# TencentARC/HOSNeRF

Hardware: AMD Instinct MI355X
Metric: train rays/sec (stage3: forward + losses + backward + gradient all-reduce + Adam; LPIPS term OFF in this line -- stages.stage3_with_lpips carries it) (higher is better)
Workload: dtype f32 (fp16/bf16 hi-lo split MFMA x3, fp32 accumulate)

## Files before the change

hosnerf_amd/csrc/hos_chain.hip:

```cpp
#include "hos_common.h"
#include "hos_gemm_common.h"

namespace {

typedef _Float16 h8 __attribute__((ext_vector_type(8)));
typedef _Float16 h2 __attribute__((ext_vector_type(2)));

constexpr int CT = 256;
constexpr int CROWS = 128;
constexpr int NL = 6;
constexpr int CW = 128;
constexpr int KSMAX = 12;
constexpr int CBUF = KSMAX * 2 * 1024;
constexpr int SKIP_LAYER = 4;

__host__ __device__ constexpr int ks_of(int l, bool fold = false) { return l == SKIP_LAYER ? 12 : ((fold && l == 0) ? 4 : 8); }
__host__ __device__ constexpr int layer_off(int l, bool fold = false) {
    int o = 0;
    for (int i = 0; i < l; ++i) o += 4 * ks_of(i, fold) * 2048;
    return o;
}
constexpr int WC_BYTES = layer_off(NL);
constexpr int W0H_LD = 64;

struct ChainArgs {
    const float* E; int lde;
    const float* PE; int ldpe;
    const float* x;
    const uint16_t* Wc;
    const float* aux;
    float* acts[NL]; int ldact;
    float* xyz;
    long P; const int* p_dev;
    unsigned int* range_flag;
};
constexpr int AUX_FLOATS = NL * CW + 3 * CW + 4;
constexpr int AUX_BYTES = (AUX_FLOATS * 4 + 15) & ~15;
constexpr int SMEM_BYTES = 2 * CBUF + AUX_BYTES;

__device__ __forceinline__ void dma16(const void* gsrc, void* ldst) {
    __builtin_amdgcn_global_load_lds((const __attribute__((address_space(1))) void*)gsrc,
                                     (__attribute__((address_space(3))) void*)ldst, 16, 0, 0);
}

__device__ __forceinline__ f32x16 mfma3(const h8& ah, const h8& al, const h8& bh, const h8& bl, f32x16 acc) {
    acc = __builtin_amdgcn_mfma_f32_32x32x16_f16(al, bh, acc, 0, 0, 0);
    acc = __builtin_amdgcn_mfma_f32_32x32x16_f16(ah, bl, acc, 0, 0, 0);
    acc = __builtin_amdgcn_mfma_f32_32x32x16_f16(ah, bh, acc, 0, 0, 0);
    return acc;
}

__device__ __forceinline__ void split_to(float x, _Float16& hi, _Float16& lo) {
    hi = (_Float16)__builtin_amdgcn_fmed3f(x, -65504.f, 65504.f);
    lo = (_Float16)(x - (float)hi);
}

__device__ __forceinline__ void load_split8(const float* p, h8& hi, h8& lo) {
    const float4 a = *reinterpret_cast<const float4*>(p);
    const float4 b = *reinterpret_cast<const float4*>(p + 8);
    const float v[8] = {a.x, a.y, a.z, a.w, b.x, b.y, b.z, b.w};
#pragma unroll
    for (int c = 0; c < 8; ++c) { _Float16 h, l; split_to(v[c], h, l); hi[c] = h; lo[c] = l; }
}

#define CH_RD128(DST, ADDR, OFF) asm volatile("ds_read_b128 %0, %1 offset:%2" : "=v"(DST) : "v"(ADDR), "n"(OFF))

template <bool FOLD>
__global__ __launch_bounds__(CT, 2) void chain128_kernel(ChainArgs a) {
    extern __shared__ __attribute__((aligned(16))) char smem[];
    char* const wbuf = smem;
    float* const s_aux = reinterpret_cast<float*>(smem + 2 * CBUF);
    const int t = threadIdx.x, lane = t & 63, wave = t >> 6;
    const int r = lane & 31, hh = lane >> 5;
    long P = a.P;
    if (a.p_dev) P = min(P, (long)*a.p_dev);
    for (int i = t; i < AUX_FLOATS; i += CT) s_aux[i] = a.aux[i];
    const long ntiles = (P + CROWS - 1) / CROWS;
    if ((long)blockIdx.x >= ntiles) return;

    const unsigned voff = (unsigned)(wave * 1024 + lane * 16);
    auto issue_round = [&](int l, int ob, int parity, int q) {
        const int ks = ks_of(l, FOLD);
        const int lo = (l * 8 + (l > SKIP_LAYER ? 4 : 0) - ((FOLD && l > 0) ? 4 : 0)) * 4 * 2048;
        dma16(reinterpret_cast<const char*>(a.Wc) + lo + ob * ks * 2048 + voff + q * 4096, wbuf + parity * CBUF + wave * 1024 + q * 4096);
    };
    auto issue_chunk = [&](int l, int ob, int parity) {
        const int rounds = ks_of(l, FOLD) / 2;
        for (int q = 0; q < rounds; ++q) issue_round(l, ob, parity, q);
    };
    issue_chunk(0, 0, 0);
    const unsigned lds_base = (unsigned)(uintptr_t)(__attribute__((address_space(3))) char*)smem;

    bool big = false;
    for (long tile = blockIdx.x; tile < ntiles; tile += gridDim.x) {
        const long row = tile * CROWS + wave * 32 + r;
        const long lrow = row < P ? row : P - 1;
        const bool tile_full = (tile + 1) * CROWS <= P;
        h8 bh[KSMAX], bl[KSMAX];
        if constexpr (FOLD) {
            const float* pe = a.PE + (size_t)lrow * a.ldpe + 4 * hh;
#pragma unroll
            for (int s = 0; s < 4; ++s) load_split8(pe + 16 * s, bh[8 + s], bl[8 + s]);
#pragma unroll
            for (int s = 0; s < 8; ++s)
#pragma unroll
                for (int c = 0; c < 8; ++c) { bh[s][c] = (_Float16)0.f; bl[s][c] = (_Float16)0.f; }
        } else {
            const float* e = a.E + (size_t)lrow * a.lde + 4 * hh;
#pragma unroll
            for (int s = 0; s < 8; ++s) load_split8(e + 16 * s, bh[s], bl[s]);
#pragma unroll
            for (int s = 8; s < KSMAX; ++s)
#pragma unroll
                for (int c = 0; c < 8; ++c) { bh[s][c] = (_Float16)0.f; bl[s][c] = (_Float16)0.f; }
        }
        float part[3] = {0.f, 0.f, 0.f};
        int parity = 0;
#pragma unroll 1
// ... 264 lines not shown
```

hosnerf_amd/csrc/hos_gemm_common.h:

```cpp
#pragma once
#include "hos_common.h"

typedef float f32x16 __attribute__((ext_vector_type(16)));

enum Mode { MODE_FWD = 0, MODE_DGRAD = 1, MODE_WGRAD = 2 };

struct GemmArgs {
    const float* A0; int lda0; int kt0;
    const float* A1; int lda1;
    const float* B;  int ldb;
    float* C; int ldc;
    int M, N;
    int Mload, Nload;
    int red_limit;
    int nk;
    int kt_per_split;
    int tiles_m, tiles_n;
    const float* bias;
    const float* mask; int ldmask;
    float* aux; int aux_col; float p0, p1;
    float* db;
    int accumulate;
    int epi;
    const int* m_dev;
// ... 75 lines not shown
                v[0] += bias4.x; v[1] += bias4.y; v[2] += bias4.z; v[3] += bias4.w;
                const bool simple = (a.epi == HOS_EPI_NONE || a.epi == HOS_EPI_RELU);
                if (relu_bits != nullptr) {
                    uint32_t rb = *relu_bits;
#pragma unroll
                    for (int k = 0; k < 4; ++k) rb = __builtin_amdgcn_alignbit(rb, __float_as_uint(0.f - v[k]), 31);
                    *relu_bits = rb;
                }
                if (simple && full && c_vec) {
                    const float pre = (v[0] + v[1]) + (v[2] + v[3]);
                    if (a.epi == HOS_EPI_RELU) { v[0] = fmaxf(v[0], 0.f); v[1] = fmaxf(v[1], 0.f); v[2] = fmaxf(v[2], 0.f); v[3] = fmaxf(v[3], 0.f); }
                    big |= (fmaxf(fmaxf(fabsf(v[0]), fabsf(v[1])), fmaxf(fabsf(v[2]), fabsf(v[3]))) > HOS_RANGE_LIMIT) | (pre != pre);
                    *reinterpret_cast<float4*>(a.C + (size_t)row * a.ldc + colb) = make_float4(v[0], v[1], v[2], v[3]);
                } else {
#pragma unroll
                    for (int k = 0; k < 4; ++k) {
                        const int col = colb + k;
                        if (col >= a.N) break;
                        float x = v[k];
                        if (fwd_epilogue_value(a, x, row, col)) a.C[(size_t)row * a.ldc + col] = x;
                        if (simple) big |= !(fabsf(x) <= HOS_RANGE_LIMIT);
                    }
                }
            } else {
                if (a.mask != nullptr) {
                    if (full && m_vec) {
                        const float4 mk = *reinterpret_cast<const float4*>(a.mask + (size_t)row * a.ldmask + colb);
                        if (!(mk.x > 0.f)) v[0] = 0.f;
                        if (!(mk.y > 0.f)) v[1] = 0.f;
                        if (!(mk.z > 0.f)) v[2] = 0.f;
                        if (!(mk.w > 0.f)) v[3] = 0.f;
                    } else {
#pragma unroll
                        for (int k = 0; k < 4; ++k)
                            if (colb + k < a.N && !(a.mask[(size_t)row * a.ldmask + colb + k] > 0.f)) v[k] = 0.f;
                    }
                }
                float* dst = a.C + (size_t)row * a.ldc + colb;
                if (full && c_vec) {
                    float4 o = make_float4(v[0], v[1], v[2], v[3]);
                    if (a.accumulate) { const float4 p = *reinterpret_cast<const float4*>(dst); o.x += p.x; o.y += p.y; o.z += p.z; o.w += p.w; }
                    *reinterpret_cast<float4*>(dst) = o;
                } else {
#pragma unroll
                    for (int k = 0; k < 4; ++k)
                        if (colb + k < a.N) dst[k] = a.accumulate ? (dst[k] + v[k]) : v[k];
                }
            }
        }
        if (MODE == MODE_FWD && a.range_flag != nullptr && __builtin_amdgcn_ballot_w64(big) != 0 && lane == 0) atomicOr(a.range_flag, 1u);
    }
}

#define HOS_GEMM_FP32 0
#define HOS_GEMM_BF16X3 1
int hos_gemm3_launch(GemmArgs a, int mode, int splits, hipStream_t stream);
```

hosnerf_amd/human_nerf.py:

```python
from __future__ import annotations

import json
import math
import os
from types import SimpleNamespace
from typing import Dict, List, Optional

import numpy as np
import torch
import torch.nn as nn
import torch.nn.functional as F

from . import ops
from .flat import FlatModule, FlatStore, Region
from .mipnerf360 import select_state, _Lin

SMPL_PARENT = {1: 0, 2: 0, 3: 0, 4: 1, 5: 2, 6: 3, 7: 4, 8: 5, 9: 6, 10: 7, 11: 8, 12: 9, 13: 9, 14: 9, 15: 12,
               16: 13, 17: 14, 18: 16, 19: 17, 20: 18, 21: 19, 22: 20, 23: 21, 24: 23, 25: 22}


class Cfg(dict):

    def __getattr__(self, k):
        try:
# ... 423 lines not shown
        ops.embed_hannw(x, band_w, cond.reshape(-1), E, PE, rows_dev=rows_dev)
        if chain:
            key = id(specs)
            bufs = self._chain_bufs.get(key)
            if bufs is None or bufs[0].device != dev:
                bufs = self._chain_bufs[key] = ops.mlp_chain_buffers(dev)
            ws = [self._w(L) for L in specs]
            ops.mlp_chain_pack([w for w, _ in ws], [b_ for _, b_ in ws], bufs[0], bufs[1])
            acts = [torch.empty(Pn, 128, device=dev) for _ in range(6)]
            xyz = torch.empty(Pn, 3, device=dev)
            ops.mlp_chain128_fwd(E, PE, x, bufs[0], bufs[1], acts, xyz, rows_dev=rows_dev)
            return xyz, ((E, PE, acts, None) if save else None)
        acts = []
        h = E
        for i in range(6):
            L = specs[i]
            Wt, bt = self._w(L)
            out = torch.empty(Pn, 128, device=dev)
            if i == 4:
                ops.linear_fwd(h, 128, Wt, bt, 128, out, ops.EPI_RELU, A1=PE, K1=NR_LDPE, rows_dev=rows_dev)
            else:
                ops.linear_fwd(h, L.Kpad, Wt, bt, 128, out, ops.EPI_RELU, rows_dev=rows_dev)
            acts.append(out)
            h = out
        Wt, bt = self._w(specs[6])
        xyz = torch.empty(Pn, 3, device=dev)
        ops.linear_fwd(h, 128, Wt, bt, 3, xyz, ops.EPI_RESIDUAL, aux=x, rows_dev=rows_dev)
        return xyz, ((E, PE, acts, None) if save else None)

    def _canonical_fwd(self, cnl: torch.Tensor, state: int, save: bool, rows_dev=None):
        Pn = cnl.shape[0]
        dev = cnl.device
        embed = self._embeds.view(self.store.param)[state]
        fold = None
        if rows_dev is not None and not ops.thin_dgrad_rows(Pn):
            raise ValueError("_canonical_fwd(rows_dev=...): the row bound exists on the thin-kernel path only (ops.thin_dgrad_rows)")
        if ops.CNL_FOLD and ops.thin_dgrad_rows(Pn):
            fkey = ("cnl_fold",) + ops._stream_key(dev)
            fb = self._chain_bufs.get(fkey)
            if fb is None:
                fb = self._chain_bufs[fkey] = torch.empty(256 * (2 * CNL_NFP + 256 + 2), device=dev)
            fw = ops.cnl_fold_views(fb, 256, CNL_NFP, 256)
            (W0, b0), (W5, b5) = self._w(self._cnl[0]), self._w(self._cnl[5])
            ops.canonical_fold_pack(W0, b0, W5, b5, embed, 256, CNL_NF, 256, fw)
            E = torch.empty(Pn, CNL_NFP, device=dev)
            CAT = torch.empty(Pn, CNL_NFP + 256, device=dev)
            ops.embed_fourier(cnl, 10, ops.zero1(dev), E, CAT, rows_dev=rows_dev)
            fold = (fw, embed)
        else:
            E = torch.empty(Pn, CNL_LDE, device=dev)
            CAT = torch.empty(Pn, CNL_CAT, device=dev)
            CAT[:, CNL_CAT - 1].zero_()
            ops.embed_fourier(cnl, 10, embed, E, CAT, rows_dev=rows_dev)
        acts, bits = [], []
        h = E
        want_bits = save and ops.thin_dgrad_rows(Pn)
        for i in range(8):
            L = self._cnl[i]
            Wt, bt = self._w(L)
            K = L.Kpad
            if fold is not None and i in (0, 5):
                Wt, bt = (fold[0][0], fold[0][1]) if i == 0 else (fold[0][2], fold[0][3])
                K = Wt.shape[1]
            rb = ops.thin_relu_bits(Pn, dev) if (want_bits and K <= 320) else None
            if i == 4:
                ops.linear_fwd(h, K, Wt, bt, 256, CAT, ops.EPI_RELU, out_col0=CNL_NFP if fold is not None else 127, relu_bits=rb,
                               rows_dev=rows_dev)
                acts.append(CAT)
                h = CAT
            else:
                out = torch.empty(Pn, 256, device=dev)
                ops.linear_fwd(h, K, Wt, bt, 256, out, ops.EPI_RELU, relu_bits=rb, rows_dev=rows_dev)
                acts.append(out)
                h = out
            bits.append(rb)
        Wt, bt = self._w(self._cnl[8])
        raw = torch.empty(Pn, 4, device=dev)
        ops.linear_fwd(h, 256, Wt, bt, 4, raw, ops.EPI_SIGMOID_RELU4, rows_dev=rows_dev)
        return raw, ((E, acts, bits, fold) if save else None)

    def _nonrigid_bwd(self, specs: List[_LayerSpec], saved, x: torch.Tensor, band_w: torch.Tensor, g_xyz: torch.Tensor, rows_dev=None):
        E, PE, acts, fold = saved
        Pn, dev = x.shape[0], x.device

        def layer_bwd(dz, X, spec, N, K, out, relu_mask, w_col0=0, bias=True, override=None):
            if override is not None:
                Wt, gW, gb = override
            else:
                Wt, _ = self._w(spec)
                gW, gb = self._w(spec, grad=True)
            ops.linear_bwd_fused(dz, X, Wt, gW, gb if bias else None, N, K, out, relu_mask, w_col0=w_col0, rows_dev=rows_dev)
            return out

        dz6 = torch.empty(Pn, 32, device=dev)
        ops.slice_pad(g_xyz, 0, 3, dz6, rows_dev=rows_dev)
        if fold is not None:
            gfold = ops.zero_(ops.fold_grad_workspace(dev))
            gw0h, db0 = gfold[:128 * 64].view(128, 64), gfold[128 * 64:]
        if (fold is not None and ops.MLP_CHAIN_BWD and Pn >= ops.MLP_CHAIN_BWD_MIN_ROWS
                and ops.get_gemm_mode() != ops.GEMM_FP32):
            Wm = [self._w(L)[0] for L in specs]
            G = [self._w(L, grad=True) for L in specs]
            im = ops.mlp_chain_bwd_images(id(specs), (0, 1, 2), dev)
            ops.mlp_chain_bwd_pack([
                (0, 0, Wm[6], 0, 3, 128, im[0][0]), (0, 1, Wm[5], 0, 128, 128, im[0][1]),
                (1, 0, Wm[4], 128, 128, NR_LDPE, im[1][0]), (1, 1, Wm[4], 0, 128, 128, im[1][1]), (1, 2, Wm[3], 0, 128, 128, im[1][2]),
# ... 302 lines not shown
```

hosnerf_amd/ops.py:

```python
from __future__ import annotations

import os
import threading

import math
from typing import Optional, Tuple

import numpy as np
import torch

from . import _lib
from ._lib import call, ptr

EPS = 1.1920929e-07

EPI_NONE, EPI_RELU, EPI_DENSITY, EPI_RGB, EPI_NERF_HEAD, EPI_SIGMOID_RELU4, EPI_RESIDUAL = 0, 1, 2, 3, 4, 5, 6


def round_up(x: int, m: int) -> int:
    return (x + m - 1) // m * m


class KernelEvents:

# ... 334 lines not shown
    import ctypes
    for i in range(0, len(jobs), 8):
        js = jobs[i:i + 8]
        Wp = (ctypes.c_void_p * len(js))(*[ptr(j[2]) + 4 * j[3] for j in js])
        call("hos_mlp_chain_bwd_pack", len(js), _int_array([j[0] for j in js]), _int_array([j[1] for j in js]), Wp,
             _int_array([j[2].stride(0) for j in js]), _int_array([j[4] for j in js]), _int_array([j[5] for j in js]),
             (ctypes.c_void_p * len(js))(*[ptr(j[6], torch.int16) for j in js]))


def mlp_chain_bwd(cfg, dZ, X, images, dXout, dW, w_col0, db, N, K, rows_dev=None):
    import ctypes
    M = dZ.shape[0]
    S = len(X)
    need = int(_lib.load().hos_mlp_chain_bwd_ws_floats(cfg, M))
    ws = _bwd_workspace(dZ.device, need=need)
    flop = sum(4.0 * M * n * k for n, k in zip(N, K))
    _timed(f"mlp_chain_bwd{cfg}[M={M}]", flop, lambda: call(
        "hos_mlp_chain_bwd", cfg, ptr(dZ), dZ.stride(0), M, ptr(rows_dev, torch.int32), _ptr_array(list(X)), _int_array([x.stride(0) for x in X]),
        (ctypes.c_void_p * S)(*[ptr(im, torch.int16) for im in images]), _ptr_array(list(dXout)),
        _int_array([0 if o is None else o.stride(0) for o in dXout]),
        (ctypes.c_void_p * S)(*[ptr(g) + 4 * c for g, c in zip(dW, w_col0)]), _int_array([g.stride(0) for g in dW]),
        _ptr_array(list(db)), _int_array(N), _int_array(K), ptr(ws), ws.numel()))


def mlp_chain_buffers(device):
    lib = _lib.load()
    return (torch.empty(int(lib.hos_mlp_chain_weight_bytes()) // 2, dtype=torch.int16, device=device),
            torch.empty(int(lib.hos_mlp_chain_aux_floats()), device=device))


def mlp_chain_pack(weights, biases, planes, aux):
    import ctypes
    ldw = (ctypes.c_int * 7)(*[int(w.stride(0)) for w in weights])
    call("hos_mlp_chain_pack", _ptr_array(list(weights)), ldw, _ptr_array(list(biases)), ptr(planes, torch.int16), ptr(aux))


def mlp_chain_pack_fold(weights, biases, cond, nfeat, planes, aux, w0h):
    import ctypes
    ldw = (ctypes.c_int * 7)(*[int(w.stride(0)) for w in weights])
    call("hos_mlp_chain_pack_fold", _ptr_array(list(weights)), ldw, _ptr_array(list(biases)), ptr(cond), cond.numel(), nfeat,
         ptr(planes, torch.int16), ptr(aux), ptr(w0h))


def mlp_chain_unfold_grad(gw0h, db, cond, nfeat, gW0, gb0):
    call("hos_mlp_chain_unfold_grad", ptr(gw0h), ptr(db), ptr(cond), cond.numel(), nfeat, ptr(gW0), gW0.stride(0), ptr(gb0))


def mlp_chain128_fwd(E, PE, x, planes, aux, acts, xyz, rows_dev=None):
    P = x.shape[0]
    flop = 101120 if E is not None else 101120 - 128 * 64
    _timed(f"mlp_chain128{'' if E is not None else 'f'}[M={P}]", 2.0 * P * flop, lambda: call(
        "hos_mlp_chain128_fwd", ptr(E), 0 if E is None else E.stride(0), ptr(PE), PE.stride(0), ptr(x), ptr(planes, torch.int16), ptr(aux),
        _ptr_array(list(acts)), acts[0].stride(0), ptr(xyz), P, ptr(rows_dev, torch.int32)))


_RANGE_FLAG = {}
RANGE_GUARD = os.environ.get("HOS_RANGE_GUARD", "1") != "0"


def arm_range_flag(device) -> torch.Tensor:
    key = str(device)
    if key not in _RANGE_FLAG:
        _RANGE_FLAG[key] = torch.zeros(1, dtype=torch.int32, device=device)
    _lib.check(_lib.load().hos_set_range_flag(ptr(_RANGE_FLAG[key], torch.int32)), "hos_set_range_flag")
    return _RANGE_FLAG[key]


def range_events(device, reset: bool = True) -> int:
    flag = _RANGE_FLAG.get(str(device))
    if flag is None:
        return 0
    v = int(flag.item())
    if v and reset:
        flag.zero_()
    return v


_RANGE_SKIPS = {}
_RANGE_SKIPS_SEEN = {}


def range_guard_words(device):
    if not RANGE_GUARD:
        return None, None
    key = str(device)
    if key not in _RANGE_FLAG or key not in _RANGE_SKIPS:
        if torch.cuda.is_current_stream_capturing():
            return None, None
        arm_range_flag(device)
        _RANGE_SKIPS[key] = torch.zeros(2, dtype=torch.int32, device=device)
    return _RANGE_FLAG[key], _RANGE_SKIPS[key]


def range_skips(device, since_last_poll: bool = False) -> int:
    key = str(device)
    t = _RANGE_SKIPS.get(key)
    if t is None:
        return 0
    n = int(t[0].item())
    if since_last_poll:
        n, _RANGE_SKIPS_SEEN[key] = n - _RANGE_SKIPS_SEEN.get(key, 0), n
    return n


def guarded_forward(module, device, run):
    mode = getattr(module, "gemm_mode", None)
# ... 1279 lines not shown
```

include/hosrender.h:

```cpp
#ifndef HOSRENDER_H
#define HOSRENDER_H

#include <stdint.h>

#ifdef __cplusplus
extern "C" {
#endif

#define HOS_OK 0
#define HOS_E_ARG (-1)
#define HOS_E_ALIGN (-2)
#define HOS_E_SHAPE (-3)
#define HOS_E_NODEVICE (-4)

typedef void* hos_stream_t;

#define HOS_ABI_VERSION 101

int hos_version(void);
int hos_device_count(void);
const char* hos_error_string(int code);


#define HOS_GEMM_MODE_FP32 0
// ... 213 lines not shown
int hos_raw2outputs_bwd(const float* g_rgb, const float* g_weights, const float* rgbs, int rgb_ld,
                        const float* sigma, int sigma_ld, const float* z_vals, const float* rays_d,
                        const float* mask, const float* bgcolor, float last_dist, int B, int S,
                        float* g_rgbs, int g_rgb_ld, float* g_sigma, int g_sigma_ld, float* g_mask,
                        hos_stream_t stream);

int hos_merge_composite_fwd(const float* bkg_tdist, const float* bkg_rgb, const float* bkg_density,
                            const float* human_rgbsigma, const float* newsmpl_pts, const float* pts_mask,
                            const float* rays_o_bkg, const float* rays_d_bkg, const float* smpl_to_world,
                            const int32_t* tiny_d_flag, int B, int Sb, int Sh, float thre_fg,
                            float* rgb, int32_t* idx_fg, int32_t* total_order, float* human_weights_sorted,
                            float* z_human, hos_stream_t stream);
int hos_merge_composite_maps_fwd(const float* bkg_tdist, const float* bkg_rgb, const float* bkg_density,
                                 const float* human_rgbsigma, const float* newsmpl_pts, const float* pts_mask,
                                 const float* rays_o_bkg, const float* rays_d_bkg, const float* smpl_to_world,
                                 const int32_t* tiny_d_flag, int B, int Sb, int Sh, float thre_fg,
                                 float* rgb, int32_t* idx_fg, int32_t* total_order,
                                 float* acc, float* depth, float* rgb_human, float* acc_human,
                                 float* rgb_bkg, float* acc_bkg, hos_stream_t stream);
int hos_merge_composite_bwd(const float* g_rgb, const float* g_human_weights_sorted,
                            const float* bkg_tdist, const float* bkg_rgb, const float* bkg_density,
                            const float* human_rgbsigma, const float* newsmpl_pts, const float* pts_mask,
                            const float* rays_o_bkg, const float* rays_d_bkg, const float* smpl_to_world,
                            const int32_t* tiny_d_flag, int B, int Sb, int Sh, float thre_fg,
                            float* g_bkg_rgb, float* g_bkg_density, float* g_human_rgbsigma, float* g_pts_mask,
                            hos_stream_t stream);

long long hos_pose_refine_saved_floats(void);
long long hos_pose_refine_workspace_floats(void);
int hos_pose_refine_fwd(const float* posevec, const float* Rs, const float* Ts, const float* const* weights14,
                        int F, int K, int width, float* Rs_out, float* Ts_out, float* saved, hos_stream_t stream);
int hos_pose_refine_bwd(const float* g_Rs_out, const float* g_Ts_out, const float* posevec, const float* Rs,
                        const float* saved, const float* const* weights14, float* const* grads14, int F, int K, int width,
                        float* workspace, hos_stream_t stream);

int hos_motion_basis_fwd(const float* dst_Rs, const float* dst_Ts, const float* cnl_gtfms, int F, int K,
                         float* R_bwd, float* T_bwd, float* R_fwd, float* T_fwd, hos_stream_t stream);
int hos_motion_basis_bwd(const float* g_R_bwd, const float* g_T_bwd, const float* g_R_fwd, const float* g_T_fwd,
                         const float* dst_Rs, const float* dst_Ts, const float* cnl_gtfms, int F, int K,
                         float* g_dst_Rs, float* g_dst_Ts, hos_stream_t stream);

long long hos_mlp_chain_weight_bytes(void);
long long hos_mlp_chain_aux_floats(void);
int hos_mlp_chain_pack(const float* const* weights7, const int* ldw7, const float* const* biases7, void* chain_planes,
                       float* aux, hos_stream_t stream);
int hos_mlp_chain_pack_fold(const float* const* weights7, const int* ldw7, const float* const* biases7, const float* cond,
                            int ncond, int nfeat, void* chain_planes, float* aux, float* w0h, hos_stream_t stream);
int hos_mlp_chain_unfold_grad(const float* gw0h, const float* db, const float* cond, int ncond, int nfeat,
                              float* gW0, int ldw, float* gb0, hos_stream_t stream);
int hos_mlp_chain128_fwd(const float* E, int lde, const float* PE, int ldpe, const float* x, const void* chain_planes,
                         const float* aux, float* const* acts6, int ldact, float* xyz, int64_t P,
                         const int32_t* rows_dev, hos_stream_t stream);

int hos_mlp_chain_bwd_steps(int cfg);
long long hos_mlp_chain_bwd_image_bytes(int cfg, int step);
long long hos_mlp_chain_bwd_ws_floats(int cfg, int M);
int hos_mlp_chain_bwd_pack(int n, const int* cfg, const int* step, const float* const* W, const int* ldw, const int* N, const int* K,
                           void* const* image, hos_stream_t stream);
int hos_mlp_chain_bwd(int cfg, const float* dZ, int lddz, int M, const int32_t* rows_dev, const float* const* X, const int* ldx,
                      const void* const* images, float* const* dXout, const int* lddx, float* const* dW, const int* lddw,
                      float* const* db, const int* N, const int* K, float* ws, int64_t ws_floats, hos_stream_t stream);

long long hos_compact_workspace_ints(void);
int hos_compact_rows(const float* mask, float thr, const float* src_a, const float* src_b, int64_t P, int32_t* count,
                     int32_t* sel, float* out_a, float* out_b, int32_t* workspace, hos_stream_t stream);
int hos_scatter_rows(const float* src, const int32_t* sel, const int32_t* count, int64_t P, float* dst, hos_stream_t stream);

int hos_select_live_rays(const float* mask, float thr, int B, int S, int32_t* ray_ids, int32_t* flag, int32_t* rows_live,
                         hos_stream_t stream);
int hos_gather_rays(const float* src, const int32_t* ray_ids, const int32_t* rows_live, int B, int S, int C, float* dst,
                    hos_stream_t stream);
int hos_scatter_rays(const float* src, const int32_t* ray_ids, const int32_t* flag, const int32_t* rows_live, int B, int S,
                     int C, float* dst, hos_stream_t stream);

long long hos_train_losses_workspace_floats(void);
int hos_train_losses_fwd(const float* rgb, const float* target, long long n_rays, float mse_const, float mse_count,
                         const float* pts_prev, const float* weights, const float* ray_grid, const int32_t* fg,
                         const float* cam_prev, const float* intrinsics_prev, int S,
                         const float* observe, const float* deform, long long n_cyc, const int32_t* n_cyc_dev,
                         float w_mse, float w_flow, float w_cycle, float* workspace, float* out8,
                         hos_stream_t stream);
int hos_train_losses_bwd(const float* g_total, const float* out8, const float* rgb, const float* target, long long n_rays,
                         float mse_count, const float* pts_prev, const float* weights, const float* ray_grid,
                         const int32_t* fg, const float* cam_prev, const float* intrinsics_prev, int S,
                         const float* observe, const float* deform, long long n_cyc, const int32_t* n_cyc_dev,
                         float w_mse, float w_flow, float w_cycle,
                         float* g_rgb, float* g_pts_prev, float* g_weights, float* g_deform, hos_stream_t stream);

int hos_sumsq(const float* g, int64_t n, float* sumsq, hos_stream_t stream);
int hos_adam_step(float* p, const float* g, float* m, float* v, int64_t n, float lr, float beta1,
                  float beta2, float eps, int step, float grad_scale, const float* sumsq,
                  float max_norm, hos_stream_t stream);

int hos_adam_step_dyn(float* p, const float* g, float* m, float* v, int64_t n, const float* hyper,
                      float beta1, float beta2, float eps, float grad_scale, const float* sumsq,
                      float max_norm, hos_stream_t stream);

int hos_rowdot_lrelu_fwd(const float* x, const float* W, int ldw, const float* b, int N, int K, float slope, float* y,
                         hos_stream_t stream);
int hos_rowdot_lrelu_bwd(const float* g, const float* y, const float* x, const float* W, int ldw, int N, int K, float slope,
                         float* gW, int ldgw, float* gb, float* gx, hos_stream_t stream);
int hos_volume_softmax_fwd(const float* z, const float* prior, int C, long long V3, float* vol, hos_stream_t stream);
int hos_volume_softmax_bwd(const float* g_vol, const float* vol, int C, long long V3, float* gz, hos_stream_t stream);
int hos_volume_channel_last(const float* vol, int Kb, long long V3, float* vol_cl, hos_stream_t stream);
int hos_volume_pair_bwd(const float* g_vol, const float* g_cl, int C, int Kb, long long V3, float* g, hos_stream_t stream);
int hos_copy_or_zero_n(int n, float* const* dst, const float* const* src, const long long* count, hos_stream_t stream);
// ... 47 lines not shown
```

Measured before the change: 143,300.

## Fuse the 8-layer canonical MLP into one persistent chain256 kernel

Adds a persistent HIP kernel that runs the full 256-wide, 8-layer canonical NeRF MLP, including the skip layer and the 4-output head, inside one launch. Activations stay in registers as fp16 hi/lo splits, and weight tiles are double-buffered into LDS with global_load_lds DMA. When saving for backward it writes activations and packed ReLU sign bits. This replaces a sequence of per-layer GEMM launches and their activation round-trips through global memory. The cost is a large single-occupancy kernel (launch_bounds 1, big LDS footprint) and a weight repack on every forward call.

```diff
diff --git a/hosnerf_amd/csrc/hos_chain.hip b/hosnerf_amd/csrc/hos_chain.hip
--- a/hosnerf_amd/csrc/hos_chain.hip
+++ b/hosnerf_amd/csrc/hos_chain.hip
@@ -3,8 +3,7 @@
 
 namespace {
 
-typedef _Float16 h8 __attribute__((ext_vector_type(8)));
-typedef _Float16 h2 __attribute__((ext_vector_type(2)));
+using namespace hos_chainp;
 
 constexpr int CT = 256;
 constexpr int CROWS = 128;
@@ -37,33 +36,6 @@
 constexpr int AUX_FLOATS = NL * CW + 3 * CW + 4;
 constexpr int AUX_BYTES = (AUX_FLOATS * 4 + 15) & ~15;
 constexpr int SMEM_BYTES = 2 * CBUF + AUX_BYTES;
-
-__device__ __forceinline__ void dma16(const void* gsrc, void* ldst) {
-    __builtin_amdgcn_global_load_lds((const __attribute__((address_space(1))) void*)gsrc,
-                                     (__attribute__((address_space(3))) void*)ldst, 16, 0, 0);
-}
-
-__device__ __forceinline__ f32x16 mfma3(const h8& ah, const h8& al, const h8& bh, const h8& bl, f32x16 acc) {
-    acc = __builtin_amdgcn_mfma_f32_32x32x16_f16(al, bh, acc, 0, 0, 0);
-    acc = __builtin_amdgcn_mfma_f32_32x32x16_f16(ah, bl, acc, 0, 0, 0);
-    acc = __builtin_amdgcn_mfma_f32_32x32x16_f16(ah, bh, acc, 0, 0, 0);
-    return acc;
-}
-
-__device__ __forceinline__ void split_to(float x, _Float16& hi, _Float16& lo) {
-    hi = (_Float16)__builtin_amdgcn_fmed3f(x, -65504.f, 65504.f);
-    lo = (_Float16)(x - (float)hi);
-}
-
-__device__ __forceinline__ void load_split8(const float* p, h8& hi, h8& lo) {
-    const float4 a = *reinterpret_cast<const float4*>(p);
-    const float4 b = *reinterpret_cast<const float4*>(p + 8);
-    const float v[8] = {a.x, a.y, a.z, a.w, b.x, b.y, b.z, b.w};
-#pragma unroll
-    for (int c = 0; c < 8; ++c) { _Float16 h, l; split_to(v[c], h, l); hi[c] = h; lo[c] = l; }
-}
-
-#define CH_RD128(DST, ADDR, OFF) asm volatile("ds_read_b128 %0, %1 offset:%2" : "=v"(DST) : "v"(ADDR), "n"(OFF))
 
 template <bool FOLD>
 __global__ __launch_bounds__(CT, 2) void chain128_kernel(ChainArgs a) {
diff --git a/hosnerf_amd/csrc/hos_chain256.hip b/hosnerf_amd/csrc/hos_chain256.hip
--- /dev/null
+++ b/hosnerf_amd/csrc/hos_chain256.hip
@@ -0,0 +1,307 @@
+#include "hos_common.h"
+#include "hos_gemm_common.h"
+
+namespace {
+
+using namespace hos_chainp;
+
+typedef float f32x4 __attribute__((ext_vector_type(4)));
+typedef unsigned u32x4 __attribute__((ext_vector_type(4)));
+
+constexpr int CT = 256;
+constexpr int CROWS = 128;
+constexpr int NL = 8;
+constexpr int CW = 256;
+constexpr int NOB = CW / 32;
+constexpr int KSE = 4;
+constexpr int KSH = CW / 16;
+constexpr int KSMAX = KSH + KSE;
+constexpr int CBUF = KSMAX * 2048;
+constexpr int SKIP_LAYER = 5;
+constexpr int NOUT = 4;
+
+__host__ __device__ constexpr int ks_of(int l) { return l == 0 ? KSE : (l == SKIP_LAYER ? KSMAX : KSH); }
+__host__ __device__ constexpr int ks_before(int l) { return l == 0 ? 0 : KSE + KSH * (l - 1) + (l > SKIP_LAYER ? KSE : 0); }
+constexpr int WC_BYTES = NOB * ks_before(NL) * 2048;
+constexpr int AUX_FLOATS = NL * CW + NOUT * CW + NOUT;
+constexpr int AUX_BYTES = (AUX_FLOATS * 4 + 15) & ~15;
+constexpr int BITS_BYTES = 4 * 1024;
+constexpr int SMEM_BYTES = 2 * CBUF + AUX_BYTES + BITS_BYTES;
+
+struct Chain256Args {
+    const float* E; int lde;
+    const uint16_t* Wc;
+    const float* aux;
+    float* acts[NL]; int ldact[NL];
+    uint16_t* bits[NL];
+    float* raw;
+    long P; const int* p_dev;
+    unsigned int* range_flag;
+};
+
+template <int NS, int CS0, int SLOT0, bool EPI, typename F, typename G, typename H>
+__device__ __forceinline__ void run_steps(f32x16& acc, const h8 (&bh)[KSMAX], const h8 (&bl)[KSMAX], unsigned la, F&& issue, H&& pre, G&& epi) {
+    h8 fh[2], fl[2];
+    f32x4 bq = {0.f, 0.f, 0.f, 0.f};
+    CH_RD128(fh[0], la, (2 * CS0) * 1024);
+    CH_RD128(fl[0], la, (2 * CS0 + 1) * 1024);
+#pragma unroll
+    for (int s = 0; s < NS; ++s) {
+        if (EPI && s >= NS - 4) pre(s - (NS - 4), bq);
+        if (s < NS - 1) {
+            CH_RD128(fh[(s + 1) & 1], la, (2 * (CS0 + s) + 2) * 1024);
+            CH_RD128(fl[(s + 1) & 1], la, (2 * (CS0 + s) + 3) * 1024);
+            asm volatile("s_waitcnt lgkmcnt(2)" : "+v"(fh[s & 1]), "+v"(fl[s & 1]), "+v"(bq));
+        } else {
+            asm volatile("s_waitcnt lgkmcnt(0)" : "+v"(fh[0]), "+v"(fl[0]), "+v"(fh[1]), "+v"(fl[1]), "+v"(bq));
+        }
+        acc = mfma3(fh[s & 1], fl[s & 1], bh[SLOT0 + s], bl[SLOT0 + s], acc);
+        issue(CS0 + s);
+        if (EPI && s >= NS - 4) epi(s - (NS - 4), bq);
+    }
+}
+
+template <bool SAVE>
+__global__ __launch_bounds__(CT, 1) void chain256_kernel(Chain256Args a) {
+    extern __shared__ __attribute__((aligned(16))) char smem[];
+    char* const wbuf = smem;
+    float* const s_aux = reinterpret_cast<float*>(smem + 2 * CBUF);
+    const int t = threadIdx.x, lane = t & 63, wave = __builtin_amdgcn_readfirstlane(t >> 6);
+    const int r = lane & 31, hh = lane >> 5;
+    long P = a.P;
+    if (a.p_dev) P = min(P, (long)*a.p_dev);
+    for (int i = t; i < AUX_FLOATS; i += CT) s_aux[i] = a.aux[i];
+    const long ntiles = (P + CROWS - 1) / CROWS;
+    if ((long)blockIdx.x >= ntiles) return;
+
+    const unsigned voff = (unsigned)(wave * 1024 + lane * 16);
+    auto issue_round = [&](int l, int ob, int parity, int q) {
+        const unsigned off = (unsigned)((NOB * ks_before(l) + ob * ks_of(l)) * 2048 + q * 4096) + voff;
+        dma16(reinterpret_cast<const char*>(a.Wc) + off, wbuf + parity * CBUF + wave * 1024 + q * 4096);
+    };
+    for (int q = 0; q < KSE / 2; ++q) issue_round(0, 0, 0, q);
+    const unsigned lds_base = (unsigned)(uintptr_t)(__attribute__((address_space(3))) char*)smem;
+
+    const int thin_l0 = 32 * ((r >> 2) & 1) + (r & 3) + 4 * hh;
+    const int bits_shift = 12 - 4 * (r >> 3) + 16 * (r & 1);
+    const unsigned bits_la = lds_base + (unsigned)(2 * CBUF + AUX_BYTES + wave * 1024 + (thin_l0 >> 1) * 4);
+    const unsigned stage_la = lds_base + (unsigned)(2 * CBUF + AUX_BYTES + wave * 1024 + lane * 16);
+
+    float v_max = 0.f, pre_sum = 0.f;
+    for (long tile = blockIdx.x; tile < ntiles; tile += gridDim.x) {
+        const long row0 = tile * CROWS + wave * 32;
+        const long row = row0 + r;
+        const long lrow = row < P ? row : P - 1;
+        const bool wave_live = row0 < P;
+        h8 bh[KSMAX], bl[KSMAX];
+        {
+            const float* e = a.E + (size_t)lrow * a.lde + 4 * hh;
+#pragma unroll
+            for (int s = 0; s < KSE; ++s) load_split8(e + 16 * s, bh[KSH + s], bl[KSH + s]);
+#pragma unroll
+            for (int s = 0; s < KSH; ++s)
+#pragma unroll
+                for (int c = 0; c < 8; ++c) { bh[s][c] = (_Float16)0.f; bl[s][c] = (_Float16)0.f; }
+        }
+        float part[NOUT] = {0.f, 0.f, 0.f, 0.f};
+        int parity = 0;
+#pragma unroll 1
+        for (int l = 0; l < NL; ++l) {
+            const int ks = ks_of(l);
+            const unsigned bias_la = lds_base + (unsigned)(2 * CBUF + (l * CW + 4 * hh) * 4);
+            float* out = SAVE ? a.acts[l] + (size_t)lrow * a.ldact[l] + 4 * hh : nullptr;
+            if (SAVE) { const u32x4 z = {0u, 0u, 0u, 0u}; asm volatile("ds_write_b128 %0, %1" :: "v"(stage_la), "v"(z) : "memory"); }
+            f32x16 acc[NOB];
+            auto epi_bias = [&](int ob, int q, f32x4& b4) {
+                asm volatile("ds_read_b128 %0, %1" : "=v"(b4) : "v"(bias_la + (unsigned)((32 * ob + 8 * q) * 4)));
+            };
+            auto epi_bias_now = [&](int ob, int q, f32x4& b4) {
+                asm volatile("ds_read_b128 %0, %1\n\ts_waitcnt lgkmcnt(0)" : "=v"(b4) : "v"(bias_la + (unsigned)((32 * ob + 8 * q) * 4)));
+            };
+            auto epi_quad = [&](f32x16& A, int ob, int q, const f32x4& b4) {
+                const int n0 = 32 * ob + 8 * q;
+                const float p0 = A[4 * q + 0] + b4[0], p1 = A[4 * q + 1] + b4[1], p2 = A[4 * q + 2] + b4[2], p3 = A[4 * q + 3] + b4[3];
+                pre_sum += (p0 + p1) + (p2 + p3);
+                const float v0 = fmaxf(p0, 0.f), v1 = fmaxf(p1, 0.f), v2 = fmaxf(p2, 0.f), v3 = fmaxf(p3, 0.f);
+                A[4 * q + 0] = v0; A[4 * q + 1] = v1; A[4 * q + 2] = v2; A[4 * q + 3] = v3;
+                v_max = fmaxf(fmaxf(v_max, fmaxf(v0, v1)), fmaxf(v2, v3));
+                if (SAVE) {
+                    uint32_t nib = 0;
+                    nib = __builtin_amdgcn_alignbit(nib, __float_as_uint(0.f - p0), 31);
+                    nib = __builtin_amdgcn_alignbit(nib, __float_as_uint(0.f - p1), 31);
+                    nib = __builtin_amdgcn_alignbit(nib, __float_as_uint(0.f - p2), 31);
+                    nib = __builtin_amdgcn_alignbit(nib, __float_as_uint(0.f - p3), 31);
+                    asm volatile("ds_or_b32 %0, %1" :: "v"(bits_la + (unsigned)(ob * 128 + q * 16)), "v"(row < P ? nib << bits_shift : 0u) : "memory");
+                    if (row < P) *reinterpret_cast<float4*>(out + n0) = make_float4(v0, v1, v2, v3);
+                }
+            };
+#pragma unroll
+            for (int ob = 0; ob < NOB; ++ob) {
+#pragma unroll
+                for (int i = 0; i < 16; ++i) acc[ob][i] = 0.f;
+                if (SAVE && wave_live && ob >= 2) asm volatile("s_waitcnt vmcnt(4)" ::: "memory");
+                else if (SAVE && wave_live && ob == 0 && l > 0) asm volatile("s_waitcnt vmcnt(8)" ::: "memory");
+                else asm volatile("s_waitcnt vmcnt(0)" ::: "memory");
+                asm volatile("s_waitcnt lgkmcnt(0)\n\ts_barrier" ::: "memory");
+                int nl = l, nob = ob + 1;
+                if (nob == NOB) { nob = 0; nl = l + 1 == NL ? 0 : l + 1; }
+                const int nrounds = ks_of(nl) / 2;
+                const int npar = parity ^ 1;
+                const unsigned la = lds_base + (unsigned)(parity * CBUF + lane * 16);
+                parity ^= 1;
+                auto issue = [&](int q) { if (q < nrounds) issue_round(nl, nob, npar, q); };
+                auto pre = [&](int q, f32x4& b4) { if (ob > 0) epi_bias(ob - 1, q, b4); };
+                auto epi = [&](int q, const f32x4& b4) {
+                    if (q == 0) asm volatile("" ::: "memory");
+                    if (ob > 0) epi_quad(acc[ob > 0 ? ob - 1 : 0], ob - 1, q, b4);
+                };
+                auto none = [](int) {};
+                auto none2 = [](int, f32x4&) {};
+                if (l == 0) {
+                    run_steps<KSE, 0, KSH, false>(acc[ob], bh, bl, la, issue, none2, none2);
+                    for (int q = KSE; q < nrounds; ++q) issue_round(nl, nob, npar, q);
+                    asm volatile("" ::: "memory");
+                    if (ob > 0) {
+#pragma unroll
+                        for (int q = 0; q < 4; ++q) { f32x4 b4; epi_bias_now(ob - 1, q, b4); epi_quad(acc[ob - 1], ob - 1, q, b4); }
+                    }
+                } else {
+                    run_steps<KSH, 0, 0, true>(acc[ob], bh, bl, la, issue, pre, epi);
+                    if (ks == KSMAX) run_steps<KSE, KSH, KSH, false>(acc[ob], bh, bl, la, none, none2, none2);
+                }
+            }
+            asm volatile("" ::: "memory");
+#pragma unroll
+            for (int q = 0; q < 4; ++q) { f32x4 b4; epi_bias_now(NOB - 1, q, b4); epi_quad(acc[NOB - 1], NOB - 1, q, b4); }
+            const bool last = l == NL - 1;
+#pragma unroll
+            for (int ob = 0; ob < NOB; ++ob) {
+#pragma unroll
+                for (int tq = 0; tq < 2; ++tq) {
+                    h8 hi, lo;
+#pragma unroll
+                    for (int c = 0; c < 8; ++c) { _Float16 h_, l_; split_to(acc[ob][8 * tq + c], h_, l_); hi[c] = h_; lo[c] = l_; }
+                    bh[2 * ob + tq] = hi;
+                    bl[2 * ob + tq] = lo;
+                }
+            }
+            if (last) {
+                const float* w8 = s_aux + NL * CW + 4 * hh;
+#pragma unroll
+                for (int ob = 0; ob < NOB; ++ob)
+#pragma unroll
+                    for (int q = 0; q < 4; ++q)
+#pragma unroll
+                        for (int m = 0; m < NOUT; ++m) {
+                            const float4 w4 = *reinterpret_cast<const float4*>(w8 + m * CW + 32 * ob + 8 * q);
+                            part[m] += acc[ob][4 * q] * w4.x + acc[ob][4 * q + 1] * w4.y + acc[ob][4 * q + 2] * w4.z + acc[ob][4 * q + 3] * w4.w;
+                        }
+            }
+            if (SAVE) {
+                u32x4 w;
+                asm volatile("ds_read_b128 %0, %1\n\ts_waitcnt lgkmcnt(0)" : "=v"(w) : "v"(stage_la) : "memory");
+                if (wave_live) *reinterpret_cast<u32x4*>(reinterpret_cast<char*>(a.bits[l]) + (size_t)(row0 / 32) * 1024 + lane * 16) = w;
+            }
+        }
+#pragma unroll
+        for (int m = 0; m < NOUT; ++m) part[m] += __shfl_xor(part[m], 32, 64);
+        if (hh == 0 && row < P) {
+            const float* b8 = s_aux + NL * CW + NOUT * CW;
+            *reinterpret_cast<float4*>(a.raw + row * 4) = make_float4(sigmoid_f(part[0] + b8[0]), sigmoid_f(part[1] + b8[1]),
+                                                                      sigmoid_f(part[2] + b8[2]), fmaxf(part[3] + b8[3], 0.f));
+        }
+    }
+    asm volatile("s_waitcnt vmcnt(0)" ::: "memory");
+    if (a.range_flag != nullptr && __builtin_amdgcn_ballot_w64((v_max > HOS_RANGE_LIMIT) | (pre_sum != pre_sum)) != 0 && lane == 0) atomicOr(a.range_flag, 1u);
+}
+
+struct Pack256Args {
+    const float* W[NL + 1]; int ldw[NL + 1];
+    const float* b[NL + 1];
+    uint16_t* Wc; float* aux;
+};
+
+__global__ __launch_bounds__(256) void chain256_pack_kernel(Pack256Args p) {
+    const int l = blockIdx.y;
+    if (l == NL) {
+        for (int i = blockIdx.x * 256 + threadIdx.x; i < AUX_FLOATS; i += gridDim.x * 256) {
+            float v;
+            if (i < NL * CW) v = p.b[i / CW][i % CW];
+            else if (i < NL * CW + NOUT * CW) { const int j = i - NL * CW; v = p.W[NL][(size_t)(j / CW) * p.ldw[NL] + j % CW]; }
+            else v = p.b[NL][i - NL * CW - NOUT * CW];
+            p.aux[i] = v;
+        }
+        return;
+    }
+    const int ks = ks_of(l);
+    const int total = NOB * ks * 64 * 8;
+    uint16_t* dst = p.Wc + (size_t)NOB * ks_before(l) * 1024;
+    for (int e = blockIdx.x * 256 + threadIdx.x; e < total; e += gridDim.x * 256) {
+        const int c = e & 7, lane = (e >> 3) & 63, s = (e >> 9) % ks, ob = (e >> 9) / ks;
+        const int n = 32 * ob + (lane & 31);
+        int k = 16 * s + 8 * (c >> 2) + 4 * (lane >> 5) + (c & 3);
+        if (l == SKIP_LAYER) k = k < CW ? k + 16 * KSE : k - CW;
+        _Float16 hi, lo;
+        split_to(p.W[l][(size_t)n * p.ldw[l] + k], hi, lo);
+        const size_t o = (((size_t)(ob * ks + s) * 2) * 64 + lane) * 8 + c;
+        dst[o] = __builtin_bit_cast(uint16_t, hi);
+        dst[o + 64 * 8] = __builtin_bit_cast(uint16_t, lo);
+    }
+}
+
+template <bool SAVE>
+int chain256_launch(const Chain256Args& a, hipStream_t stream) {
+    static bool attr_set = false;
+    if (!attr_set) {
+        hipError_t e = hipFuncSetAttribute(reinterpret_cast<const void*>(&chain256_kernel<SAVE>), hipFuncAttributeMaxDynamicSharedMemorySize, SMEM_BYTES);
+        if (e != hipSuccess) return (int)e;
+        attr_set = true;
+    }
+    const long ntiles = (a.P + CROWS - 1) / CROWS;
+    constexpr int max_grid = 256;
+    const int grid = (int)(ntiles < max_grid ? ntiles : max_grid);
+    hipLaunchKernelGGL(chain256_kernel<SAVE>, dim3(grid), dim3(CT), SMEM_BYTES, stream, a);
+    return hos_launch_status();
+}
+
+}
+
+extern "C" long long hos_mlp_chain256_weight_bytes(void) { return WC_BYTES; }
+extern "C" long long hos_mlp_chain256_aux_floats(void) { return AUX_FLOATS; }
+
+extern "C" int hos_mlp_chain256_pack(const float* const* weights9, const int* ldw9, const float* const* biases9, void* chain_planes,
+                                     float* aux, hos_stream_t stream) {
+    if (!weights9 || !ldw9 || !biases9 || !chain_planes || !aux) return HOS_E_ARG;
+    Pack256Args p{};
+    for (int l = 0; l <= NL; ++l) {
+        if (!weights9[l] || !biases9[l]) return HOS_E_ARG;
+        if (ldw9[l] < (l == NL ? CW : 16 * ks_of(l))) return HOS_E_SHAPE;
+        p.W[l] = weights9[l]; p.ldw[l] = ldw9[l]; p.b[l] = biases9[l];
+    }
+    p.Wc = static_cast<uint16_t*>(chain_planes); p.aux = aux;
+    hipLaunchKernelGGL(chain256_pack_kernel, dim3(48, NL + 1), dim3(256), 0, static_cast<hipStream_t>(stream), p);
+    return hos_launch_status();
+}
+
+extern "C" int hos_mlp_chain256_canonical_fwd(const float* E, int lde, const void* chain_planes, const float* aux,
+                                              float* const* acts8, const int* ldact8, void* const* relu_bits8, float* raw,
+                                              int64_t P, const int32_t* rows_dev, hos_stream_t stream) {
+    if (!E || !chain_planes || !aux || !raw || P <= 0) return HOS_E_ARG;
+    if (lde < 16 * KSE || P > (int64_t)1 << 22) return HOS_E_SHAPE;
+    if ((lde & 3) || (((uintptr_t)E | (uintptr_t)chain_planes | (uintptr_t)raw) & 15u)) return HOS_E_ALIGN;
+    Chain256Args a{};
+    a.E = E; a.lde = lde; a.Wc = static_cast<const uint16_t*>(chain_planes); a.aux = aux; a.raw = raw;
+    a.P = P; a.p_dev = rows_dev; a.range_flag = hos_range_flag_ptr();
+    const bool save = acts8 != nullptr;
+    if (save) {
+        if (!ldact8 || !relu_bits8) return HOS_E_ARG;
+        for (int l = 0; l < NL; ++l) {
+            if (!acts8[l] || !relu_bits8[l]) return HOS_E_ARG;
+            if (ldact8[l] < CW) return HOS_E_SHAPE;
+            if ((ldact8[l] & 3) || (((uintptr_t)acts8[l] | (uintptr_t)relu_bits8[l]) & 15u)) return HOS_E_ALIGN;
+            a.acts[l] = acts8[l]; a.ldact[l] = ldact8[l]; a.bits[l] = static_cast<uint16_t*>(relu_bits8[l]);
+        }
+    }
+    hipStream_t s = static_cast<hipStream_t>(stream);
+    return save ? chain256_launch<true>(a, s) : chain256_launch<false>(a, s);
+}
diff --git a/hosnerf_amd/csrc/hos_gemm_common.h b/hosnerf_amd/csrc/hos_gemm_common.h
--- a/hosnerf_amd/csrc/hos_gemm_common.h
+++ b/hosnerf_amd/csrc/hos_gemm_common.h
@@ -151,6 +151,40 @@
     }
 }
 
+namespace hos_chainp {
+
+typedef _Float16 h8 __attribute__((ext_vector_type(8)));
+typedef _Float16 h2 __attribute__((ext_vector_type(2)));
+
+__device__ __forceinline__ void dma16(const void* gsrc, void* ldst) {
+    __builtin_amdgcn_global_load_lds((const __attribute__((address_space(1))) void*)gsrc,
+                                     (__attribute__((address_space(3))) void*)ldst, 16, 0, 0);
+}
+
+__device__ __forceinline__ f32x16 mfma3(const h8& ah, const h8& al, const h8& bh, const h8& bl, f32x16 acc) {
+    acc = __builtin_amdgcn_mfma_f32_32x32x16_f16(al, bh, acc, 0, 0, 0);
+    acc = __builtin_amdgcn_mfma_f32_32x32x16_f16(ah, bl, acc, 0, 0, 0);
+    acc = __builtin_amdgcn_mfma_f32_32x32x16_f16(ah, bh, acc, 0, 0, 0);
+    return acc;
+}
+
+__device__ __forceinline__ void split_to(float x, _Float16& hi, _Float16& lo) {
+    hi = (_Float16)__builtin_amdgcn_fmed3f(x, -65504.f, 65504.f);
+    lo = (_Float16)(x - (float)hi);
+}
+
+__device__ __forceinline__ void load_split8(const float* p, h8& hi, h8& lo) {
+    const float4 a = *reinterpret_cast<const float4*>(p);
+    const float4 b = *reinterpret_cast<const float4*>(p + 8);
+    const float v[8] = {a.x, a.y, a.z, a.w, b.x, b.y, b.z, b.w};
+#pragma unroll
+    for (int c = 0; c < 8; ++c) { _Float16 h, l; split_to(v[c], h, l); hi[c] = h; lo[c] = l; }
+}
+
+#define CH_RD128(DST, ADDR, OFF) asm volatile("ds_read_b128 %0, %1 offset:%2" : "=v"(DST) : "v"(ADDR), "n"(OFF))
+
+}
+
 #define HOS_GEMM_FP32 0
 #define HOS_GEMM_BF16X3 1
 int hos_gemm3_launch(GemmArgs a, int mode, int splits, hipStream_t stream);
diff --git a/hosnerf_amd/human_nerf.py b/hosnerf_amd/human_nerf.py
--- a/hosnerf_amd/human_nerf.py
+++ b/hosnerf_amd/human_nerf.py
@@ -499,6 +499,23 @@
             CAT = torch.empty(Pn, CNL_CAT, device=dev)
             CAT[:, CNL_CAT - 1].zero_()
             ops.embed_fourier(cnl, 10, embed, E, CAT, rows_dev=rows_dev)
+        if fold is not None and ops.mlp_chain256_rows(Pn):
+            ckey = ("cnl_chain256",) + ops._stream_key(dev)
+            cb = self._chain_bufs.get(ckey)
+            if cb is None:
+                cb = self._chain_bufs[ckey] = ops.mlp_chain256_buffers(dev)
+            ws = [self._w(L) for L in self._cnl]
+            ws[0], ws[5] = (fold[0][0], fold[0][1]), (fold[0][2], fold[0][3])
+            ops.mlp_chain256_pack([w for w, _ in ws], [b_ for _, b_ in ws], cb[0], cb[1])
+            raw = torch.empty(Pn, 4, device=dev)
+            if not save:
+                ops.mlp_chain256_canonical_fwd(E, cb[0], cb[1], raw, rows_dev=rows_dev)
+                return raw, None
+            acts = [CAT if i == 4 else torch.empty(Pn, 256, device=dev) for i in range(8)]
+            bits = [ops.thin_relu_bits(Pn, dev) for _ in range(8)]
+            ops.mlp_chain256_canonical_fwd(E, cb[0], cb[1], raw, acts, bits, act_col0=[CNL_NFP if i == 4 else 0 for i in range(8)],
+                                           rows_dev=rows_dev)
+            return raw, (E, acts, bits, fold)
         acts, bits = [], []
         h = E
         want_bits = save and ops.thin_dgrad_rows(Pn)
diff --git a/hosnerf_amd/ops.py b/hosnerf_amd/ops.py
--- a/hosnerf_amd/ops.py
+++ b/hosnerf_amd/ops.py
@@ -410,6 +410,45 @@
     _timed(f"mlp_chain128{'' if E is not None else 'f'}[M={P}]", 2.0 * P * flop, lambda: call(
         "hos_mlp_chain128_fwd", ptr(E), 0 if E is None else E.stride(0), ptr(PE), PE.stride(0), ptr(x), ptr(planes, torch.int16), ptr(aux),
         _ptr_array(list(acts)), acts[0].stride(0), ptr(xyz), P, ptr(rows_dev, torch.int32)))
+
+
+MLP_CHAIN256 = True
+MLP_CHAIN256_MIN_ROWS = 16384
+
+
+def mlp_chain256_rows(M: int) -> bool:
+    return bool(MLP_CHAIN256 and CNL_FOLD and M >= MLP_CHAIN256_MIN_ROWS and thin_dgrad_rows(M)
+                and get_gemm_mode() in (GEMM_PLANES, GEMM_BF16X3))
+
+
+def mlp_chain256_buffers(device):
+    lib = _lib.load()
+    return (torch.empty(int(lib.hos_mlp_chain256_weight_bytes()) // 2, dtype=torch.int16, device=device),
+            torch.empty(int(lib.hos_mlp_chain256_aux_floats()), device=device))
+
+
+def mlp_chain256_pack(weights, biases, planes, aux):
+    import ctypes
+    ldw = (ctypes.c_int * 9)(*[int(w.stride(0)) for w in weights])
+    call("hos_mlp_chain256_pack", _ptr_array(list(weights)), ldw, _ptr_array(list(biases)), ptr(planes, torch.int16), ptr(aux))
+
+
+def mlp_chain256_canonical_fwd(E, planes, aux, raw, acts=None, bits=None, act_col0=None, rows_dev=None):
+    import ctypes
+    P = E.shape[0]
+    flop = 2.0 * P * (64 * 256 + 6 * 256 * 256 + 320 * 256 + 256 * 4)
+    if acts is None:
+        _timed(f"mlp_chain256_cnl[M={P}]", flop, lambda: call(
+            "hos_mlp_chain256_canonical_fwd", ptr(E), E.stride(0), ptr(planes, torch.int16), ptr(aux), None, None, None, ptr(raw), P,
+            ptr(rows_dev, torch.int32)))
+        return
+    ld = (ctypes.c_int * 8)(*[int(t.stride(0)) for t in acts])
+    bp = (ctypes.c_void_p * 8)(*[ptr(b, torch.int16) for b in bits])
+    c0 = [0] * 8 if act_col0 is None else act_col0
+    ap = (ctypes.c_void_p * 8)(*[ptr(t) + 4 * int(c) for t, c in zip(acts, c0)])
+    _timed(f"mlp_chain256_cnl_save[M={P}]", flop, lambda: call(
+        "hos_mlp_chain256_canonical_fwd", ptr(E), E.stride(0), ptr(planes, torch.int16), ptr(aux), ap, ld, bp,
+        ptr(raw), P, ptr(rows_dev, torch.int32)))
 
 
 _RANGE_FLAG = {}
diff --git a/include/hosrender.h b/include/hosrender.h
--- a/include/hosrender.h
+++ b/include/hosrender.h
@@ -289,6 +289,14 @@
                          const float* aux, float* const* acts6, int ldact, float* xyz, int64_t P,
                          const int32_t* rows_dev, hos_stream_t stream);
 
+long long hos_mlp_chain256_weight_bytes(void);
+long long hos_mlp_chain256_aux_floats(void);
+int hos_mlp_chain256_pack(const float* const* weights9, const int* ldw9, const float* const* biases9, void* chain_planes,
+                          float* aux, hos_stream_t stream);
+int hos_mlp_chain256_canonical_fwd(const float* E, int lde, const void* chain_planes, const float* aux,
+                                   float* const* acts8, const int* ldact8, void* const* relu_bits8, float* raw,
+                                   int64_t P, const int32_t* rows_dev, hos_stream_t stream);
+
 int hos_mlp_chain_bwd_steps(int cfg);
 long long hos_mlp_chain_bwd_image_bytes(int cfg, int step);
 long long hos_mlp_chain_bwd_ws_floats(int cfg, int M);
```

New measurement: 144,100, median of 6. No clear change (+0.6%).
